# rhymes-ai/Aria

Hardware: NVIDIA H100
Metric: Aria-25.3B bf16 prefill tokens/sec (higher is better)
Workload: dtype bf16

## Files before the change

### aria_b200/csrc/gemm.cu

```cuda
#include <cuda_fp8.h>

#include "gemm_common.cuh"

namespace aria {

constexpr int GEMM_STAGES = 4;
constexpr int FP8_LAND_STAGES = 3;
constexpr int FP8_CONVERT_WARPS = 3;
constexpr int PAIR_MIN_ROWS = 2048;
constexpr int WIDE_PAIR_MIN_K = 2048;
template <int BN, bool B_FP8 = false>
constexpr int gemm_smem_bytes() {
  return 1024  + GEMM_STAGES * (A_STAGE_BYTES + BN * BK * 2) + BM * acc_ld(BN) * 4 + 256  +
         (B_FP8 ? FP8_LAND_STAGES * BN * BK : 0);
}
static_assert(gemm_smem_bytes<128, true>() <= 232448, "fp8 landing ring must fit the opt-in shared memory of a block");

ARIA_DEVICE void e4m3x16_to_bf16(const uint4 v, uint4& lo, uint4& hi) {
  const uint32_t w[4] = {v.x, v.y, v.z, v.w};
  uint32_t o[8];
#pragma unroll
  for (int i = 0; i < 4; ++i) {
#pragma unroll
    for (int h = 0; h < 2; ++h) {
      const __half2_raw hr = __nv_cvt_fp8x2_to_halfraw2(static_cast<__nv_fp8x2_storage_t>(w[i] >> (16 * h)), __NV_E4M3);
      const float2 f = __half22float2(__half2(hr));
      o[2 * i + h] = pack_bf16(f.x, f.y);
    }
  }
  lo = make_uint4(o[0], o[1], o[2], o[3]);
  hi = make_uint4(o[4], o[5], o[6], o[7]);
}

template <bool PAIR> ARIA_DEVICE int first_tile() { return PAIR ? blockIdx.x >> 1 : blockIdx.x; }
template <bool PAIR> ARIA_DEVICE int tile_step() { return PAIR ? gridDim.x >> 1 : gridDim.x; }
template <bool PAIR> ARIA_DEVICE int pair_sched_n(int n_tiles) { return PAIR ? (n_tiles + 1) / 2 : n_tiles; }

template <int BN, bool B_MN>
ARIA_DEVICE void wgmma_tile_k16(float (&acc)[BN / 2], uint64_t da, uint64_t db) {
  if constexpr (BN == 128) wgmma_m64n128_ss<0, B_MN ? 1 : 0>(acc, da, db, 1u);
  else wgmma_m64n144_ss<0, B_MN ? 1 : 0>(acc, da, db, 1u);
}

// ... 199 lines not shown
        const uint64_t db = db0 + rp.stage * (STAGE_BYTES >> 4);
        wgmma_fence();
#pragma unroll
        for (int k = 0; k < BK / 16; ++k) wgmma_tile_k16<BN, B_MN>(acc, da + k * 2, db + k * b_kadv);
        wgmma_commit();
        wgmma_wait<1>();
        if (prev >= 0) release(prev);
        prev = static_cast<int>(rp.stage);
        rp.next();
      }
      wgmma_wait<0>();
      fence_regs(acc);
      if (prev >= 0) release(prev);
      stage_and_epilogue<BN, EPI, B_FP8 ? AccScale::COL : AccScale::NONE>(p, stg, ct, acc, bsc, 1.f, 1.f, n_out_total, grp,
                                                                           m_idx, n_idx, row0, rows);
    }
  }
  if constexpr (PAIR) cluster_sync();
}

constexpr int WIDE_BN = 192;
constexpr int WIDE_STAGE_BYTES = A_STAGE_BYTES + WIDE_BN * BK * 2;
constexpr int WIDE_BOX_BYTES = 64 * 64 * 2;
constexpr int WIDE_HALF_BYTES = 3 * WIDE_BOX_BYTES;
constexpr int gemm_wide_smem_bytes() {
  return 1024  + GEMM_STAGES * WIDE_STAGE_BYTES + 2 * WIDE_HALF_BYTES + 256 ;
}
static_assert(gemm_wide_smem_bytes() <= 232448, "wide GEMM must fit the opt-in shared memory of a block");

ARIA_DEVICE uint32_t wide_out_offset(int r, int c) {
  return (c >> 6) * WIDE_BOX_BYTES + r * 128 + ((((c & 63) >> 3) ^ (r & 7)) << 4) + (c & 7) * 2;
}

template <int EPI, bool PAIR>
__global__ void __launch_bounds__(GEMM_THREADS, 1)
gemm_wide_kernel(const __grid_constant__ CUtensorMap tmA, const __grid_constant__ CUtensorMap tmB0,
                 const __grid_constant__ CUtensorMap tmB1, const __grid_constant__ CUtensorMap tmB2,
                 const __grid_constant__ CUtensorMap tmOut, const __grid_constant__ CUtensorMap tmRes, const GemmParams p) {
  constexpr int BN = WIDE_BN;
  constexpr int STAGES = GEMM_STAGES;
  static_assert(EPI == ARIA_EPI_LINEAR || EPI == ARIA_EPI_HEADS, "wide GEMM epilogues");

  uint8_t* smem = smem_1024();
  uint8_t* out_tile = smem + STAGES * WIDE_STAGE_BYTES;
  const BarrierRing<STAGES> bar(out_tile + 2 * WIDE_HALF_BYTES);
  uint64_t* res_full = bar.empty + STAGES;
  uint64_t* out_free = res_full + 2;

  const int warp = threadIdx.x >> 5;
  const int lane = threadIdx.x & 31;
  const int wg = threadIdx.x >> 7;
  const bool res = EPI == ARIA_EPI_LINEAR && p.residual != nullptr;

  if (warp == 0 && lane == 0) {
    prefetch_tmap(&tmA);
    prefetch_tmap(&tmB0);
    if (p.n_seg > 1) prefetch_tmap(&tmB1);
    if (p.n_seg > 2) prefetch_tmap(&tmB2);
    if (EPI == ARIA_EPI_LINEAR) prefetch_tmap(&tmOut);
    if (res) prefetch_tmap(&tmRes);
    bar.init(1, PAIR ? 2 * CONSUMER_WARPS : CONSUMER_WARPS);
    for (int h = 0; h < 2; ++h) {
      mbar_init(&res_full[h], 1);
      mbar_init(&out_free[h], 1);
    }
    fence_mbar_init();
  }
  if constexpr (PAIR) cluster_sync();
  else __syncthreads();

  const int n_out_total = p.N * p.n_seg;
  const int n_tiles = (n_out_total + BN - 1) / BN;
  const int k_blocks = (p.K + BK - 1) / BK;
  const uint32_t smem_base = smem_u32(smem);
  const uint32_t full0 = smem_u32(bar.full), empty0 = smem_u32(bar.empty);
  auto tile_boxes = [&](int col0) { return min(3, (n_out_total - col0 + 63) / 64); };

  if (wg == 0) {
    setmaxnreg_dec<56>();
    if (warp == 0 && elect_one()) {
      const uint32_t rank = PAIR ? cluster_ctarank() : 0;
      TileSched sched;
      sched.init(p, pair_sched_n<PAIR>(n_tiles));
      RingPos<STAGES> rp;
      uint32_t out_phase = 0;
      for (int t = first_tile<PAIR>();; t += tile_step<PAIR>()) {
        int grp, m_idx, n_idx, row0, rows;
        if (!sched.decode(t, grp, m_idx, n_idx, row0, rows)) break;
        if constexpr (PAIR) n_idx = 2 * n_idx + rank;
        const bool phantom = PAIR && n_idx >= n_tiles;
        const int a_row = m_idx * BM;
        const int a_half_row = a_row + (a_row + static_cast<int>(rank) * (BM / 2) < rows ? rank * (BM / 2) : 0);
        const int col0 = n_idx * BN;
        const int seg = col0 / p.N;
        const CUtensorMap* tb = seg == 0 ? &tmB0 : (seg == 1 ? &tmB1 : &tmB2);
        const int b_row = col0 - seg * p.N;
        const int res_kb = min(STAGES - 1, k_blocks - 1);
        for (int kb = 0; kb < k_blocks; ++kb) {
          const uint32_t fb = full0 + rp.stage * 8;
          const uint32_t sa = smem_base + rp.stage * WIDE_STAGE_BYTES;
          mbar_wait_addr(empty0 + rp.stage * 8, rp.phase ^ 1);
          if constexpr (PAIR) {
            mbar_arrive_expect_tx_addr(fb, phantom ? A_STAGE_BYTES : WIDE_STAGE_BYTES);
            tma_load_2d_multicast_addr(sa + rank * (A_STAGE_BYTES / 2), &tmA, fb, kb * BK, a_half_row, 0b11);
            if (phantom) {
              rp.next();
              continue;
            }
          } else {
            mbar_arrive_expect_tx_addr(fb, WIDE_STAGE_BYTES);
            tma_load_2d_addr(sa, &tmA, fb, kb * BK, a_row);
          }
          tma_load_2d_addr(sa + A_STAGE_BYTES, tb, fb, kb * BK, b_row);
          rp.next();
          if (res && kb == res_kb) {
            const int nbox = tile_boxes(col0);
            for (int h = 0; h < 2; ++h) {
              if (a_row + 64 * h >= rows) continue;
              mbar_wait(&out_free[h], (out_phase >> h) & 1);
              out_phase ^= 1u << h;
              mbar_arrive_expect_tx(&res_full[h], nbox * WIDE_BOX_BYTES);
              for (int c = 0; c < nbox; ++c)
                tma_load_2d(out_tile + h * WIDE_HALF_BYTES + c * WIDE_BOX_BYTES, &tmRes, &res_full[h], col0 + 64 * c,
                            a_row + 64 * h);
            }
          }
        }
      }
    }
  } else {
    setmaxnreg_inc<224>();
    const int cw = wg - 1;
    const uint64_t da0 = make_smem_desc(smem_base + cw * 64 * 128, 16, 1024);
    const uint64_t db0 = make_smem_desc(smem_base + A_STAGE_BYTES, 16, 1024);
    const ConsumerThread ct = consumer_thread(cw, lane);
    const int fr = ct.frag_row - 64 * cw;
    const bool leader = (threadIdx.x & 127) == 0;
    uint8_t* half = out_tile + cw * WIDE_HALF_BYTES;
    const uint32_t rank = PAIR ? cluster_ctarank() : 0;
    TileSched sched;
    sched.init(p, pair_sched_n<PAIR>(n_tiles));
    RingPos<STAGES> rp;
    uint32_t res_phase = 0;
    auto release = [&](int s) {
      if (lane == 0) {
        mbar_arrive(&bar.empty[s]);
        if constexpr (PAIR) mbar_arrive_cluster(&bar.empty[s], rank ^ 1);
      }
    };
    auto pass_tile = [&] {
      for (int kb = 0; kb < k_blocks; ++kb) {
        mbar_wait_addr(full0 + rp.stage * 8, rp.phase);
        release(rp.stage);
        rp.next();
      }
    };
    for (int t = first_tile<PAIR>();; t += tile_step<PAIR>()) {
      int grp, m_idx, n_idx, row0, rows;
      if (!sched.decode(t, grp, m_idx, n_idx, row0, rows)) break;
      if constexpr (PAIR) n_idx = 2 * n_idx + rank;
      if (sits_out((PAIR && n_idx >= n_tiles) || m_idx * BM + 64 * cw >= rows)) {
        pass_tile();
        continue;
      }
      const int col0 = n_idx * BN;
      const int seg = col0 / p.N;
      const int cseg0 = col0 - seg * p.N;
      const __nv_bfloat16* bias = p.bias[seg];
      uint32_t bias2[BN / 8];
#pragma unroll
      for (int j = 0; j < BN / 8; ++j) {
        const int c = cseg0 + 8 * j + ct.frag_col;
        bias2[j] = (bias && c < p.N) ? __ldg(reinterpret_cast<const uint32_t*>(bias + c)) : 0u;
      }
      float acc[BN / 2];
#pragma unroll
      for (int i = 0; i < BN / 2; ++i) acc[i] = 0.f;
      int prev = -1;
      for (int kb = 0; kb < k_blocks; ++kb) {
        mbar_wait_addr(full0 + rp.stage * 8, rp.phase);
        const uint64_t da = da0 + rp.stage * (WIDE_STAGE_BYTES >> 4);
        const uint64_t db = db0 + rp.stage * (WIDE_STAGE_BYTES >> 4);
        wgmma_fence();
#pragma unroll
        for (int k = 0; k < BK / 16; ++k) wgmma_m64n192_ss<0, 0>(acc, da + k * 2, db + k * 2, 1u);
        wgmma_commit();
        if (kb == 0 && leader) {
          bulk_wait_group_read<0>();
          if (res) mbar_arrive(&out_free[cw]);
        }
        wgmma_wait<1>();
        if (prev >= 0) release(prev);
        prev = static_cast<int>(rp.stage);
        rp.next();
      }
      wgmma_wait<0>();
      fence_regs(acc);
      if (prev >= 0) release(prev);
      if (res) {
        mbar_wait(&res_full[cw], res_phase);
        res_phase ^= 1;
      }
      named_bar_sync(1 + cw, 128);
#pragma unroll
      for (int j = 0; j < BN / 8; ++j) {
        const int c = 8 * j + ct.frag_col;
#pragma unroll
        for (int i = 0; i < 2; ++i) {
          uint32_t* dst = reinterpret_cast<uint32_t*>(half + wide_out_offset(fr + 8 * i, c));
          float x0 = acc[4 * j + 2 * i], x1 = acc[4 * j + 2 * i + 1];
          if (bias) {
            x0 += bf16_lo(bias2[j]);
            x1 += bf16_hi(bias2[j]);
          }
          if constexpr (EPI == ARIA_EPI_LINEAR) {
            x0 = bf16r(x0);
            x1 = bf16r(x1);
            if (p.act != ARIA_ACT_NONE) {
              x0 = bf16r(act_apply(x0, p.act));
              x1 = bf16r(act_apply(x1, p.act));
            }
            if (res) {
              const uint32_t r = *dst;
              x0 += bf16_lo(r);
              x1 += bf16_hi(r);
            }
          }
          *dst = pack_bf16(x0, x1);
        }
        if (j % 8 == 7) asm volatile("" ::: "memory");
      }
      if constexpr (EPI == ARIA_EPI_LINEAR) {
        fence_proxy_async_smem();
        named_bar_sync(1 + cw, 128);
        if (leader) {
          const int nbox = tile_boxes(col0);
          for (int c = 0; c < nbox; ++c)
            tma_store_2d_addr(&tmOut, smem_u32(half + c * WIDE_BOX_BYTES), col0 + 64 * c, m_idx * BM + 64 * cw);
          bulk_commit_group();
        }
      } else {
        named_bar_sync(1 + cw, 128);
        constexpr int CH = BN / 8;
#pragma unroll 1
        for (int i = threadIdx.x & 127; i < 64 * CH; i += 128) {
          const int r = i / CH, c = (i % CH) * 8;
          const int r_in_grp = m_idx * BM + 64 * cw + r;
          const int cs = cseg0 + c;
          if (r_in_grp >= rows || cs + 8 > p.N) continue;
          const uint4 v = *reinterpret_cast<const uint4*>(half + wide_out_offset(r, c));
          const int b = r_in_grp / p.rows_per_batch, tok = r_in_grp - b * p.rows_per_batch;
          const int head = cs / p.head_dim, d = cs - head * p.head_dim;
          *reinterpret_cast<uint4*>(p.out[seg] + b * p.stride_b + static_cast<int64_t>(p.pos0 + tok) * p.head_ld +
                                    head * p.stride_h + d) = v;
        }
      }
    }
    if (leader) bulk_wait_group_read<0>();
  }
  if constexpr (PAIR) cluster_sync();
}

constexpr int W8_BK = 128;
static_assert(BM * W8_BK == A_STAGE_BYTES, "W8A8 A stage = bf16 A stage");

struct W8a8DenseScales {
  const float* b[3];
};

template <int BN, int EPI>
ARIA_DEVICE void load_dense_col_scales(const GemmParams& p, const W8a8DenseScales& sc, int n_idx, int frag_col,
                                       float2 (&bsc)[BN / 8]) {
#pragma unroll
  for (int j = 0; j < BN / 8; ++j) {
    int col, seg;
    if constexpr (EPI == ARIA_EPI_SWIGLU) {
      seg = 8 * j < BN / 2 ? 0 : 1;
      col = n_idx * (BN / 2) + 8 * j - seg * (BN / 2) + frag_col;
    } else {
      seg = n_idx * BN / p.N;
      col = n_idx * BN - seg * p.N + 8 * j + frag_col;
    }
    const float* srow = seg == 0 ? sc.b[0] : (seg == 1 ? sc.b[1] : sc.b[2]);
    bsc[j] = col < p.N ? __ldg(reinterpret_cast<const float2*>(srow + col)) : make_float2(0.f, 0.f);
  }
}

template <int EPI, bool DENSE>
ARIA_DEVICE void w8a8_body(const CUtensorMap* tmA, const CUtensorMap* tmA_min, const CUtensorMap* tmB0, const CUtensorMap* tmB1,
                           const CUtensorMap* tmB2, const GemmParams& p, const float* __restrict__ a_scale,
                           const W8a8DenseScales& dsc) {
  constexpr int BN = 128;
  constexpr int STAGE_BYTES = A_STAGE_BYTES + BN * W8_BK;
  constexpr int STAGES = GEMM_STAGES;
  constexpr int ACC_LD = acc_ld(BN);
// ... 219 lines not shown
    ARIA_CHECK_ARG(d->n_seg == 1);
    ARIA_CHECK_ARG(d->k % BK == 0 || (d->num_groups == 1 && d->group_mod == 0));
    ARIA_CHECK_ARG(d->n % 64 == 0);
    ARIA_CHECK_ARG(d->epilogue != ARIA_EPI_HEADS);
  } else {
    ARIA_CHECK_ARG(d->num_groups == 1 || d->n_seg == 1);
    if (swiglu) ARIA_CHECK_ARG(d->n_seg == 2 && d->b[1]);
    if (b_gnk) ARIA_CHECK_ARG(d->n_seg == 1 && !swiglu && d->epilogue == ARIA_EPI_LINEAR && d->n % 128 == 0);
    else ARIA_CHECK_ARG(d->num_groups == 1);
  }
  if (d->num_groups > 1) ARIA_CHECK_ARG(d->group_offsets != nullptr);
  if (d->group_counts) ARIA_CHECK_ARG(d->group_offsets != nullptr);
  if (d->out_group_base) ARIA_CHECK_ARG(d->out_group_row0 != nullptr && d->epilogue == ARIA_EPI_LINEAR && d->group_offsets != nullptr);
  ARIA_CHECK_ARG(d->a_rows == 0 || d->a_rows >= d->m);

  int BN = 128;
  if (d->epilogue == ARIA_EPI_HEADS) {
    ARIA_CHECK_ARG(d->head_dim > 0 && d->head_dim % 8 == 0 && d->head_ld >= d->head_dim && d->n % d->head_dim == 0);
    if (d->rope_mask) ARIA_CHECK_ARG(d->head_dim == 128 && d->rope_cos && d->rope_sin);
    if (d->n % 128 != 0) {
      ARIA_CHECK_ARG(!d->rope_mask && d->n % 144 == 0);
      BN = 144;
    }
    for (int s = 0; s < d->n_seg; ++s) ARIA_CHECK_ARG(d->out[s] && d->b[s]);
  } else {
    if (swiglu) ARIA_CHECK_ARG(d->n % 64 == 0);
    if (d->n_seg > 1 && !swiglu) ARIA_CHECK_ARG(d->n % BN == 0);
  }

  const bool dense = !b_scale && d->b_layout == ARIA_B_NK && d->num_groups == 1 && !d->group_offsets;
  const bool wide = dense && d->m >= PAIR_MIN_ROWS && (d->n_seg == 1 || d->n % WIDE_BN == 0) &&
                    (d->epilogue == ARIA_EPI_HEADS ? !d->rope_mask : d->epilogue == ARIA_EPI_LINEAR);
  const bool wide_pair = wide && d->epilogue == ARIA_EPI_LINEAR && d->k >= WIDE_PAIR_MIN_K;
  const bool pair = !wide && dense && d->epilogue == ARIA_EPI_LINEAR && d->m >= PAIR_MIN_ROWS;
  const bool half_a = wide_pair || pair;

  CUtensorMap tmA, tmA_min, tmB[3];
  const uint64_t a_buf_rows = d->a_rows > 0 ? d->a_rows : d->m;
  int rc = make_tmap_2d(&tmA, d->a, d->k, a_buf_rows, d->lda * 2, BK, half_a ? BM / 2 : BM);
  if (rc) return rc;
  tmA_min = tmA;
  if (d->group_offsets) {
    rc = make_tmap_2d(&tmA_min, d->a, d->k, a_buf_rows, d->lda * 2, BK, A_BOX_MIN);
    if (rc) return rc;
  }
  if (b_mn) {
    const uint64_t ncols = swiglu ? 2 * d->n : d->n;
    const uint64_t n_weights = d->group_mod > 0 ? d->group_mod : (d->group_mod < 0 ? d->num_groups / (-d->group_mod) : d->num_groups);
    rc = b_scale ? make_tmap_2d(&tmB[0], d->b[0], ncols, n_weights * d->k, ncols, 64, BK, CU_TENSOR_MAP_SWIZZLE_NONE,
                                CU_TENSOR_MAP_DATA_TYPE_UINT8)
                 : make_tmap_2d(&tmB[0], d->b[0], ncols, n_weights * d->k, ncols * 2, 64, BK);
    if (rc) return rc;
    tmB[1] = tmB[0];
    tmB[2] = tmB[0];
  } else {
    const int nb = swiglu ? 2 : d->n_seg;
    const uint32_t box_rows = swiglu ? BN / 2 : (wide ? WIDE_BN : BN);
    for (int s = 0; s < 3; ++s) {
      const void* ptr = s < nb ? d->b[s] : d->b[0];
      const uint64_t b_rows = b_gnk ? static_cast<uint64_t>(d->group_mod > 0 ? d->group_mod : (d->group_mod < 0 ? d->num_groups / (-d->group_mod) : d->num_groups)) * d->n : d->n;
      rc = make_tmap_2d(&tmB[s], ptr, d->k, b_rows, d->k * 2, BK, box_rows);
      if (rc) return rc;
    }
  }

  const GemmParams p = gemm_params(d, b_scale);
  if (wide) {
    CUtensorMap tmOut = tmA, tmRes = tmA;
    const uint64_t n_out = d->n * d->n_seg;
    if (d->epilogue == ARIA_EPI_LINEAR) {
      rc = make_tmap_2d(&tmOut, d->out[0], n_out, d->m, d->ldo * 2, 64, 64);
      if (rc) return rc;
      if (d->residual) {
        rc = make_tmap_2d(&tmRes, d->residual, n_out, d->m, d->ldr * 2, 64, 64);
        if (rc) return rc;
      }
    }
    const int64_t m_tiles = (d->m + BM - 1) / BM, n_tiles = (n_out + WIDE_BN - 1) / WIDE_BN;
    if (wide_pair)
      return launch_persistent_pairs<gemm_wide_kernel<ARIA_EPI_LINEAR, true>>("gemm_wide_kernel", GEMM_THREADS,
                                                                              gemm_wide_smem_bytes(), (n_tiles + 1) / 2 * m_tiles,
                                                                              stream, tmA, tmB[0], tmB[1], tmB[2], tmOut, tmRes, p);
#define ARIA_LAUNCH_WIDE(EPI_)                                                                                                \
  return launch_persistent<gemm_wide_kernel<EPI_, false>>("gemm_wide_kernel", GEMM_THREADS, gemm_wide_smem_bytes(),         \
                                                          n_tiles * m_tiles, stream, tmA, tmB[0], tmB[1], tmB[2], tmOut, tmRes, p)
    if (d->epilogue == ARIA_EPI_HEADS) ARIA_LAUNCH_WIDE(ARIA_EPI_HEADS);
    ARIA_LAUNCH_WIDE(ARIA_EPI_LINEAR);
#undef ARIA_LAUNCH_WIDE
  }
  const int64_t tiles = max_tiles(d, BN, d->num_groups > 1 ? d->num_groups : 0);
  if (pair) {
    const int64_t m_tiles = (d->m + BM - 1) / BM, pairs = (tiles / m_tiles + 1) / 2 * m_tiles;
    return launch_persistent_pairs<gemm_kernel<128, false, ARIA_EPI_LINEAR, false, true>>(
        "gemm_kernel", GEMM_THREADS, gemm_smem_bytes<128>(), pairs, stream, tmA, tmA_min, tmB[0], tmB[1], tmB[2], p);
  }
#define ARIA_LAUNCH(BN_, MN_, EPI_, ...)                                                                                     \
  return launch_persistent<gemm_kernel<BN_, MN_, EPI_, ##__VA_ARGS__>>("gemm_kernel", GEMM_THREADS,                          \
                                                                       gemm_smem_bytes<BN_, ##__VA_ARGS__>(), tiles, stream, \
                                                                       tmA, tmA_min, tmB[0], tmB[1], tmB[2], p)
  if (b_scale) {
    if (swiglu) ARIA_LAUNCH(128, true, ARIA_EPI_SWIGLU, true);
    ARIA_LAUNCH(128, true, ARIA_EPI_LINEAR, true);
  }
  if (d->epilogue == ARIA_EPI_HEADS) {
    if (BN == 128) ARIA_LAUNCH(128, false, ARIA_EPI_HEADS);
    ARIA_LAUNCH(144, false, ARIA_EPI_HEADS);
  }
  if (swiglu) {
    if (b_mn) ARIA_LAUNCH(128, true, ARIA_EPI_SWIGLU);
    ARIA_LAUNCH(128, false, ARIA_EPI_SWIGLU);
  }
  if (b_mn) ARIA_LAUNCH(128, true, ARIA_EPI_LINEAR);
  ARIA_LAUNCH(128, false, ARIA_EPI_LINEAR);
#undef ARIA_LAUNCH
}

extern "C" int aria_gemm(const aria_gemm_desc_t* d, aria_stream_t stream) {
  return gemm_run(d, nullptr, reinterpret_cast<cudaStream_t>(stream));
}

// ... 112 lines not shown
```

### aria_b200/csrc/ptx.cuh

```cuda
#pragma once
#include <cuda.h>
#include <cuda_bf16.h>
#include <cuda_runtime.h>
#include <stdint.h>

namespace aria {

#define ARIA_DEVICE __device__ __forceinline__

ARIA_DEVICE uint32_t smem_u32(const void* p) { return static_cast<uint32_t>(__cvta_generic_to_shared(p)); }

ARIA_DEVICE uint32_t elect_one() {
  uint32_t pred = 0;
  asm volatile(
      "{\n\t.reg .pred P;\n\t"
      "elect.sync _|P, 0xffffffff;\n\t"
      "selp.b32 %0, 1, 0, P;\n\t}\n"
      : "=r"(pred));
  return pred;
}

ARIA_DEVICE void mbar_init(uint64_t* bar, uint32_t count) {
  asm volatile("mbarrier.init.shared::cta.b64 [%0], %1;" ::"r"(smem_u32(bar)), "r"(count));
}
ARIA_DEVICE void fence_mbar_init() { asm volatile("fence.mbarrier_init.release.cluster;" ::: "memory"); }
ARIA_DEVICE void fence_proxy_async_smem() { asm volatile("fence.proxy.async.shared::cta;" ::: "memory"); }

ARIA_DEVICE void mbar_arrive_expect_tx(uint64_t* bar, uint32_t bytes) {
  asm volatile("mbarrier.arrive.expect_tx.shared::cta.b64 _, [%0], %1;" ::"r"(smem_u32(bar)), "r"(bytes)
               : "memory");
}
ARIA_DEVICE void mbar_arrive(uint64_t* bar) {
  asm volatile("mbarrier.arrive.shared::cta.b64 _, [%0];" ::"r"(smem_u32(bar)) : "memory");
}
ARIA_DEVICE bool mbar_try_wait(uint64_t* bar, uint32_t parity) {
  uint32_t ok;
  asm volatile(
      "{\n\t.reg .pred P;\n\t"
      "mbarrier.try_wait.parity.shared::cta.b64 P, [%1], %2;\n\t"
      "selp.b32 %0, 1, 0, P;\n\t}\n"
      : "=r"(ok) : "r"(smem_u32(bar)), "r"(parity) : "memory");
  return ok != 0;
}
ARIA_DEVICE void mbar_wait_addr(uint32_t addr, uint32_t parity) {
  uint32_t ok = 0;
  long long t0 = 0;
  for (uint32_t spin = 0;; ++spin) {
    asm volatile(
        "{\n\t.reg .pred P;\n\t"
        "mbarrier.try_wait.parity.shared::cta.b64 P, [%1], %2;\n\t"
        "selp.b32 %0, 1, 0, P;\n\t}\n"
        : "=r"(ok) : "r"(addr), "r"(parity) : "memory");
    if (ok) return;
    if ((spin & 0xFFF) == 0xFFF) {
      const long long now = clock64();
      if (t0 == 0) t0 = now;
      if (now - t0 > 4000000000ll) __trap();
    }
  }
}
ARIA_DEVICE void mbar_wait(uint64_t* bar, uint32_t parity) { mbar_wait_addr(smem_u32(bar), parity); }
ARIA_DEVICE void mbar_arrive_expect_tx_addr(uint32_t bar_addr, uint32_t bytes) {
  asm volatile("mbarrier.arrive.expect_tx.shared::cta.b64 _, [%0], %1;" ::"r"(bar_addr), "r"(bytes) : "memory");
}
ARIA_DEVICE void mbar_arrive_cluster(uint64_t* bar, uint32_t cta) {
  asm volatile(
      "{\n\t.reg .b32 ra;\n\t"
      "mapa.shared::cluster.u32 ra, %0, %1;\n\t"
      "mbarrier.arrive.shared::cluster.b64 _, [ra];\n\t}\n" ::"r"(smem_u32(bar)), "r"(cta)
      : "memory");
}

ARIA_DEVICE uint32_t cluster_ctarank() {
  uint32_t r;
  asm volatile("mov.u32 %0, %%cluster_ctarank;" : "=r"(r));
  return r;
}
ARIA_DEVICE void cluster_sync() {
  asm volatile("barrier.cluster.arrive.release;\n\tbarrier.cluster.wait.acquire;" ::: "memory");
}

ARIA_DEVICE void tma_load_2d_addr(uint32_t dst, const CUtensorMap* m, uint32_t bar_addr, int c0, int c1) {
  asm volatile(
      "cp.async.bulk.tensor.2d.shared::cluster.global.mbarrier::complete_tx::bytes [%0], [%1, {%3, %4}], [%2];"
      ::"r"(dst), "l"(reinterpret_cast<uint64_t>(m)), "r"(bar_addr), "r"(c0), "r"(c1)
      : "memory");
}
ARIA_DEVICE void tma_load_2d_multicast_addr(uint32_t dst, const CUtensorMap* m, uint32_t bar_addr, int c0, int c1,
                                            uint16_t cta_mask) {
  asm volatile(
      "cp.async.bulk.tensor.2d.shared::cluster.global.mbarrier::complete_tx::bytes.multicast::cluster [%0], [%1, {%3, %4}], [%2], %5;"
      ::"r"(dst), "l"(reinterpret_cast<uint64_t>(m)), "r"(bar_addr), "r"(c0), "r"(c1), "h"(cta_mask)
      : "memory");
}
ARIA_DEVICE void tma_store_2d_addr(const CUtensorMap* m, uint32_t src, int c0, int c1) {
  asm volatile("cp.async.bulk.tensor.2d.global.shared::cta.bulk_group [%0, {%2, %3}], [%1];"
               ::"l"(reinterpret_cast<uint64_t>(m)), "r"(src), "r"(c0), "r"(c1)
               : "memory");
}
ARIA_DEVICE void bulk_commit_group() { asm volatile("cp.async.bulk.commit_group;" ::: "memory"); }
template <int N> ARIA_DEVICE void bulk_wait_group_read() { asm volatile("cp.async.bulk.wait_group.read %0;" ::"n"(N) : "memory"); }
ARIA_DEVICE void prefetch_tmap(const CUtensorMap* m) {
  asm volatile("prefetch.tensormap [%0];" ::"l"(reinterpret_cast<uint64_t>(m)) : "memory");
}
ARIA_DEVICE void tma_load_2d(void* dst, const CUtensorMap* m, uint64_t* bar, int c0, int c1) {
// ... 144 lines not shown
```

Baseline: 19230.

## Add ping-pong warpgroup GEMM kernel for wide dense projections with moderate K

Adds a persistent ping-pong GEMM kernel in which two consumer warpgroups alternate tiles. Each warpgroup computes a full 128x128 tile while the other runs its epilogue, with named barriers handing over mainloop turns. It is routed to wide dense GEMMs that don't qualify for the wide-pair path, have at least 2048 output columns, and have A up to 24MB. The aim is to hide epilogue cost (bias, activation, residual, TMA store) behind the tensor-core mainloop. In exchange it adds a new code path with more complex synchronisation and smaller N tiles than the existing wide kernel.

Measured after the change: 19640, median of 6. +2.1%, better.

```diff
diff --git a/aria_b200/csrc/gemm.cu b/aria_b200/csrc/gemm.cu
--- a/aria_b200/csrc/gemm.cu
+++ b/aria_b200/csrc/gemm.cu
@@ -1,4 +1,6 @@
 #include <cuda_fp8.h>
+
+#include <type_traits>
 
 #include "gemm_common.cuh"
 
@@ -9,6 +11,8 @@
 constexpr int FP8_CONVERT_WARPS = 3;
 constexpr int PAIR_MIN_ROWS = 2048;
 constexpr int WIDE_PAIR_MIN_K = 2048;
+constexpr int PINGPONG_MIN_COLS = 2048;
+constexpr int64_t PINGPONG_MAX_A_BYTES = 24 << 20;
 template <int BN, bool B_FP8 = false>
 constexpr int gemm_smem_bytes() {
   return 1024  + GEMM_STAGES * (A_STAGE_BYTES + BN * BK * 2) + BM * acc_ld(BN) * 4 + 256  +
@@ -503,6 +507,229 @@
   if constexpr (PAIR) cluster_sync();
 }
 
+constexpr int PP_BN = 128;
+constexpr int PP_STAGES = 5;
+constexpr int PP_STAGE_BYTES = A_STAGE_BYTES + PP_BN * BK * 2;
+constexpr int PP_TILE_BYTES = 2 * 2 * WIDE_BOX_BYTES;
+constexpr int PP_BAR_TURN = 3;
+constexpr int gemm_pingpong_smem_bytes() {
+  return 1024  + PP_STAGES * PP_STAGE_BYTES + 2 * PP_TILE_BYTES + 256 ;
+}
+static_assert(gemm_pingpong_smem_bytes() <= 232448, "ping-pong GEMM must fit the opt-in shared memory of a block");
+
+ARIA_DEVICE uint32_t pp_out_offset(int r, int c) { return (r >> 6) * (2 * WIDE_BOX_BYTES) + wide_out_offset(r & 63, c); }
+
+template <int EPI, int ACT>
+__global__ void __launch_bounds__(GEMM_THREADS, 1)
+gemm_pingpong_kernel(const __grid_constant__ CUtensorMap tmA, const __grid_constant__ CUtensorMap tmB0,
+                     const __grid_constant__ CUtensorMap tmB1, const __grid_constant__ CUtensorMap tmB2,
+                     const __grid_constant__ CUtensorMap tmOut, const __grid_constant__ CUtensorMap tmRes, const GemmParams p) {
+  constexpr int BN = PP_BN;
+  constexpr int STAGES = PP_STAGES;
+  static_assert(EPI == ARIA_EPI_LINEAR || (EPI == ARIA_EPI_HEADS && ACT == ARIA_ACT_NONE), "ping-pong GEMM epilogues");
+
+  uint8_t* smem = smem_1024();
+  uint8_t* out_tile = smem + STAGES * PP_STAGE_BYTES;
+  const BarrierRing<STAGES> bar(out_tile + 2 * PP_TILE_BYTES);
+  uint64_t* res_full = bar.empty + STAGES;
+  uint64_t* out_free = res_full + 2;
+
+  const int warp = threadIdx.x >> 5;
+  const int lane = threadIdx.x & 31;
+  const int wg = threadIdx.x >> 7;
+  const bool res = EPI == ARIA_EPI_LINEAR && p.residual != nullptr;
+
+  if (warp == 0 && lane == 0) {
+    prefetch_tmap(&tmA);
+    prefetch_tmap(&tmB0);
+    if (p.n_seg > 1) prefetch_tmap(&tmB1);
+    if (p.n_seg > 2) prefetch_tmap(&tmB2);
+    if (EPI == ARIA_EPI_LINEAR) prefetch_tmap(&tmOut);
+    if (res) prefetch_tmap(&tmRes);
+    bar.init(1, CONSUMER_WARPS / 2);
+    for (int w = 0; w < 2; ++w) {
+      mbar_init(&res_full[w], 1);
+      mbar_init(&out_free[w], 1);
+    }
+    fence_mbar_init();
+  }
+  __syncthreads();
+
+  const int n_out_total = p.N * p.n_seg;
+  const int m_tiles = (p.M + BM - 1) / BM;
+  const int tiles = (n_out_total + BN - 1) / BN * m_tiles;
+  const int k_blocks = (p.K + BK - 1) / BK;
+  const uint32_t smem_base = smem_u32(smem);
+  const uint32_t full0 = smem_u32(bar.full), empty0 = smem_u32(bar.empty);
+  auto tile_boxes = [&](int col0) { return min(2, (n_out_total - col0 + 63) / 64); };
+
+  if (wg == 0) {
+    setmaxnreg_dec<40>();
+    if (warp == 0 && elect_one()) {
+      RingPos<STAGES> rp;
+      uint32_t out_phase = 0;
+      for (int i = 0, t = blockIdx.x; t < tiles; ++i, t += gridDim.x) {
+        const int n_idx = t / m_tiles, m_idx = t - n_idx * m_tiles;
+        const int a_row = m_idx * BM;
+        const int halves = a_row + 64 < p.M ? 2 : 1;
+        const int col0 = n_idx * BN;
+        const int seg = col0 / p.N;
+        const CUtensorMap* tb = seg == 0 ? &tmB0 : (seg == 1 ? &tmB1 : &tmB2);
+        const int b_row = col0 - seg * p.N;
+        const int res_kb = min(STAGES - 1, k_blocks - 1);
+        for (int kb = 0; kb < k_blocks; ++kb) {
+          const uint32_t fb = full0 + rp.stage * 8;
+          const uint32_t sa = smem_base + rp.stage * PP_STAGE_BYTES;
+          mbar_wait_addr(empty0 + rp.stage * 8, rp.phase ^ 1);
+          mbar_arrive_expect_tx_addr(fb, PP_STAGE_BYTES);
+          tma_load_2d_addr(sa, &tmA, fb, kb * BK, a_row);
+          tma_load_2d_addr(sa + A_STAGE_BYTES, tb, fb, kb * BK, b_row);
+          rp.next();
+          if (res && kb == res_kb) {
+            const int w = i & 1, nbox = tile_boxes(col0);
+            mbar_wait(&out_free[w], (out_phase >> w) & 1);
+            out_phase ^= 1u << w;
+            mbar_arrive_expect_tx(&res_full[w], halves * nbox * WIDE_BOX_BYTES);
+            for (int h = 0; h < halves; ++h)
+              for (int c = 0; c < nbox; ++c)
+                tma_load_2d(out_tile + w * PP_TILE_BYTES + (2 * h + c) * WIDE_BOX_BYTES, &tmRes, &res_full[w],
+                            col0 + 64 * c, a_row + 64 * h);
+          }
+        }
+      }
+    }
+  } else {
+    setmaxnreg_inc<232>();
+    const int cw = wg - 1;
+    const uint64_t da0 = make_smem_desc(smem_base, 16, 1024);
+    const uint64_t db0 = make_smem_desc(smem_base + A_STAGE_BYTES, 16, 1024);
+    constexpr uint32_t A_HALF = (64 * 128) >> 4;
+    const ConsumerThread ct = consumer_thread(0, lane);
+    const int fr = ct.frag_row;
+    const bool leader = (threadIdx.x & 127) == 0;
+    const uint32_t tile = smem_u32(out_tile + cw * PP_TILE_BYTES);
+    RingPos<STAGES> rp;
+    auto release = [&](int s) {
+      if (lane == 0) mbar_arrive(&bar.empty[s]);
+    };
+    for (int i = 0, t = blockIdx.x; t < tiles; ++i, t += gridDim.x) {
+      if ((i & 1) != cw) {
+        for (int kb = 0; kb < k_blocks; ++kb) rp.next();
+        continue;
+      }
+      const int n_idx = t / m_tiles, m_idx = t - n_idx * m_tiles;
+      const bool hi = m_idx * BM + 64 < p.M;
+      const int col0 = n_idx * BN;
+      const int seg = col0 / p.N;
+      const int cseg0 = col0 - seg * p.N;
+      float acc[2][BN / 2];
+#pragma unroll
+      for (int h = 0; h < 2; ++h)
+#pragma unroll
+        for (int j = 0; j < BN / 2; ++j) acc[h][j] = 0.f;
+      if (i > 0) named_bar_sync(PP_BAR_TURN + cw, 256);
+      auto mainloop = [&](auto HI) {
+        int prev = -1;
+        for (int kb = 0; kb < k_blocks; ++kb) {
+          mbar_wait_addr(full0 + rp.stage * 8, rp.phase);
+          const uint64_t da = da0 + rp.stage * (PP_STAGE_BYTES >> 4);
+          const uint64_t db = db0 + rp.stage * (PP_STAGE_BYTES >> 4);
+          wgmma_fence();
+#pragma unroll
+          for (int k = 0; k < BK / 16; ++k) {
+            wgmma_m64n128_ss<0, 0>(acc[0], da + k * 2, db + k * 2, 1u);
+            if constexpr (decltype(HI)::value) wgmma_m64n128_ss<0, 0>(acc[1], da + A_HALF + k * 2, db + k * 2, 1u);
+          }
+          wgmma_commit();
+          if (kb == 0 && leader) {
+            bulk_wait_group_read<0>();
+            if (res) mbar_arrive(&out_free[cw]);
+          }
+          wgmma_wait<1>();
+          if (prev >= 0) release(prev);
+          prev = static_cast<int>(rp.stage);
+          rp.next();
+        }
+        if (t + static_cast<int>(gridDim.x) < tiles) named_bar_arrive(PP_BAR_TURN + (cw ^ 1), 256);
+        wgmma_wait<0>();
+        fence_regs(acc[0]);
+        fence_regs(acc[1]);
+        if (prev >= 0) release(prev);
+      };
+      if (hi) mainloop(std::true_type{});
+      else mainloop(std::false_type{});
+      const __nv_bfloat16* bias = p.bias[seg];
+      uint32_t bias2[BN / 8];
+#pragma unroll
+      for (int j = 0; j < BN / 8; ++j) {
+        const int c = cseg0 + 8 * j + ct.frag_col;
+        bias2[j] = (bias && c < p.N) ? __ldg(reinterpret_cast<const uint32_t*>(bias + c)) : 0u;
+      }
+      if (res) mbar_wait(&res_full[cw], (i >> 1) & 1);
+      named_bar_sync(1 + cw, 128);
+#pragma unroll
+      for (int h = 0; h < 2; ++h) {
+        if (h == 1 && !hi) break;
+#pragma unroll
+        for (int j = 0; j < BN / 8; ++j) {
+          const int c = 8 * j + ct.frag_col;
+#pragma unroll
+          for (int e = 0; e < 2; ++e) {
+            const uint32_t dst = tile + pp_out_offset(64 * h + fr + 8 * e, c);
+            float x0 = acc[h][4 * j + 2 * e], x1 = acc[h][4 * j + 2 * e + 1];
+            if (bias) {
+              x0 += bf16_lo(bias2[j]);
+              x1 += bf16_hi(bias2[j]);
+            }
+            if constexpr (EPI == ARIA_EPI_LINEAR) {
+              bf16r2(x0, x1);
+              if constexpr (ACT != ARIA_ACT_NONE) {
+                x0 = act_apply(x0, ACT);
+                x1 = act_apply(x1, ACT);
+                bf16r2(x0, x1);
+              }
+              if (res) {
+                const uint32_t r = ld_shared_b32(dst);
+                x0 += bf16_lo(r);
+                x1 += bf16_hi(r);
+              }
+            }
+            st_shared_b32(dst, pack_bf16(x0, x1));
+          }
+          if (j % 8 == 7) asm volatile("" ::: "memory");
+        }
+      }
+      if constexpr (EPI == ARIA_EPI_LINEAR) {
+        fence_proxy_async_smem();
+        named_bar_sync(1 + cw, 128);
+        if (leader) {
+          const int nbox = tile_boxes(col0);
+          for (int h = 0; h < (hi ? 2 : 1); ++h)
+            for (int c = 0; c < nbox; ++c)
+              tma_store_2d_addr(&tmOut, tile + (2 * h + c) * WIDE_BOX_BYTES, col0 + 64 * c, m_idx * BM + 64 * h);
+          bulk_commit_group();
+        }
+      } else {
+        named_bar_sync(1 + cw, 128);
+        constexpr int CH = BN / 8;
+#pragma unroll 1
+        for (int q = threadIdx.x & 127; q < BM * CH; q += 128) {
+          const int r = q / CH, c = (q % CH) * 8;
+          const int r_in_grp = m_idx * BM + r;
+          const int cs = cseg0 + c;
+          if (r_in_grp >= p.M || cs + 8 > p.N) continue;
+          const uint4 v = ld_shared_v4(tile + pp_out_offset(r, c));
+          const int b = r_in_grp / p.rows_per_batch, tok = r_in_grp - b * p.rows_per_batch;
+          const int head = cs / p.head_dim, d = cs - head * p.head_dim;
+          *reinterpret_cast<uint4*>(p.out[seg] + b * p.stride_b + static_cast<int64_t>(p.pos0 + tok) * p.head_ld +
+                                    head * p.stride_h + d) = v;
+        }
+      }
+    }
+    if (leader) bulk_wait_group_read<0>();
+  }
+}
+
 constexpr int W8_BK = 128;
 static_assert(BM * W8_BK == A_STAGE_BYTES, "W8A8 A stage = bf16 A stage");
 
@@ -788,6 +1015,8 @@
   const bool wide = dense && d->m >= PAIR_MIN_ROWS && (d->n_seg == 1 || d->n % WIDE_BN == 0) &&
                     (d->epilogue == ARIA_EPI_HEADS ? !d->rope_mask : d->epilogue == ARIA_EPI_LINEAR);
   const bool wide_pair = wide && d->epilogue == ARIA_EPI_LINEAR && d->k >= WIDE_PAIR_MIN_K;
+  const bool pingpong = wide && !wide_pair && d->n * d->n_seg >= PINGPONG_MIN_COLS && (d->n_seg == 1 || d->n % PP_BN == 0) &&
+                        d->m * d->k * 2 <= PINGPONG_MAX_A_BYTES;
   const bool pair = !wide && dense && d->epilogue == ARIA_EPI_LINEAR && d->m >= PAIR_MIN_ROWS;
   const bool half_a = wide_pair || pair;
 
@@ -811,7 +1040,7 @@
     tmB[2] = tmB[0];
   } else {
     const int nb = swiglu ? 2 : d->n_seg;
-    const uint32_t box_rows = swiglu ? BN / 2 : (wide ? WIDE_BN : BN);
+    const uint32_t box_rows = swiglu ? BN / 2 : (pingpong ? PP_BN : (wide ? WIDE_BN : BN));
     for (int s = 0; s < 3; ++s) {
       const void* ptr = s < nb ? d->b[s] : d->b[0];
       const uint64_t b_rows = b_gnk ? static_cast<uint64_t>(d->group_mod > 0 ? d->group_mod : (d->group_mod < 0 ? d->num_groups / (-d->group_mod) : d->num_groups)) * d->n : d->n;
@@ -833,6 +1062,17 @@
       }
     }
     const int64_t m_tiles = (d->m + BM - 1) / BM, n_tiles = (n_out + WIDE_BN - 1) / WIDE_BN;
+    if (pingpong) {
+      const int64_t tiles = (n_out + PP_BN - 1) / PP_BN * m_tiles;
+#define ARIA_LAUNCH_PP(EPI_, ACT_)                                                                                             \
+  return launch_persistent<gemm_pingpong_kernel<EPI_, ACT_>>("gemm_pingpong_kernel", GEMM_THREADS, gemm_pingpong_smem_bytes(), \
+                                                             tiles, stream, tmA, tmB[0], tmB[1], tmB[2], tmOut, tmRes, p)
+      if (d->epilogue == ARIA_EPI_HEADS) ARIA_LAUNCH_PP(ARIA_EPI_HEADS, ARIA_ACT_NONE);
+      if (d->act == ARIA_ACT_GELU_TANH) ARIA_LAUNCH_PP(ARIA_EPI_LINEAR, ARIA_ACT_GELU_TANH);
+      if (d->act == ARIA_ACT_GELU_NEW) ARIA_LAUNCH_PP(ARIA_EPI_LINEAR, ARIA_ACT_GELU_NEW);
+      ARIA_LAUNCH_PP(ARIA_EPI_LINEAR, ARIA_ACT_NONE);
+#undef ARIA_LAUNCH_PP
+    }
     if (wide_pair)
       return launch_persistent_pairs<gemm_wide_kernel<ARIA_EPI_LINEAR, true>>("gemm_wide_kernel", GEMM_THREADS,
                                                                               gemm_wide_smem_bytes(), (n_tiles + 1) / 2 * m_tiles,
diff --git a/aria_b200/csrc/ptx.cuh b/aria_b200/csrc/ptx.cuh
--- a/aria_b200/csrc/ptx.cuh
+++ b/aria_b200/csrc/ptx.cuh
@@ -71,6 +71,18 @@
       : "memory");
 }
 
+ARIA_DEVICE void st_shared_b32(uint32_t addr, uint32_t v) { asm volatile("st.shared.b32 [%0], %1;" ::"r"(addr), "r"(v)); }
+ARIA_DEVICE uint32_t ld_shared_b32(uint32_t addr) {
+  uint32_t v;
+  asm volatile("ld.shared.b32 %0, [%1];" : "=r"(v) : "r"(addr));
+  return v;
+}
+ARIA_DEVICE uint4 ld_shared_v4(uint32_t addr) {
+  uint4 v;
+  asm volatile("ld.shared.v4.b32 {%0, %1, %2, %3}, [%4];" : "=r"(v.x), "=r"(v.y), "=r"(v.z), "=r"(v.w) : "r"(addr));
+  return v;
+}
+
 ARIA_DEVICE uint32_t cluster_ctarank() {
   uint32_t r;
   asm volatile("mov.u32 %0, %%cluster_ctarank;" : "=r"(r));
```

## Hand off wide GEMM epilogue to idle producer warps via out_full barriers

Applied to the files above, without the earlier changes.

For wide GEMM launches without a residual, the consumer warpgroups now only write bias-added bf16 accumulators into the shared-memory output tile and signal an out_full barrier. The three otherwise idle producer-warpgroup warps then apply GELU in place, issue the TMA stores, or scatter the HEADS layout to global memory. The aim is to overlap epilogue work (activation, stores) with the next tile's MMA main loop. In exchange it adds barrier round-trips and makes consumers wait on out_free before writing. Epilogue throughput is limited to 96 threads running with a reduced register budget. GELU is now applied to the bf16-rounded stored value, which matches the old rounding order.

Measured after the change: 19270 before, 19860 after (median of 6 runs). +3.1%, better.

```diff
diff --git a/aria_b200/csrc/gemm.cu b/aria_b200/csrc/gemm.cu
--- a/aria_b200/csrc/gemm.cu
+++ b/aria_b200/csrc/gemm.cu
@@ -274,7 +274,29 @@
   return (c >> 6) * WIDE_BOX_BYTES + r * 128 + ((((c & 63) >> 3) ^ (r & 7)) << 4) + (c & 7) * 2;
 }
 
-template <int EPI, bool PAIR>
+constexpr int WIDE_EPI_THREADS = 96;
+constexpr uint32_t WIDE_EPI_BAR = 3;
+
+template <int ACT>
+ARIA_DEVICE void wide_act_inplace(uint32_t half, int n_chunks, int et) {
+  auto act8 = [](uint4& v) {
+    uint32_t* w = reinterpret_cast<uint32_t*>(&v);
+#pragma unroll
+    for (int e = 0; e < 4; ++e) w[e] = pack_bf16(bf16r(act_apply(bf16_lo(w[e]), ACT)), bf16r(act_apply(bf16_hi(w[e]), ACT)));
+  };
+#pragma unroll 1
+  for (int i = et; i < n_chunks; i += 2 * WIDE_EPI_THREADS) {
+    const uint32_t a0 = half + 16 * i, a1 = a0 + 16 * WIDE_EPI_THREADS;
+    const bool two = i + WIDE_EPI_THREADS < n_chunks;
+    uint4 v0 = ld_shared_v4(a0), v1 = two ? ld_shared_v4(a1) : make_uint4(0, 0, 0, 0);
+    act8(v0);
+    act8(v1);
+    st_shared_v4(a0, v0);
+    if (two) st_shared_v4(a1, v1);
+  }
+}
+
+template <int EPI, bool PAIR, bool HANDOFF>
 __global__ void __launch_bounds__(GEMM_THREADS, 1)
 gemm_wide_kernel(const __grid_constant__ CUtensorMap tmA, const __grid_constant__ CUtensorMap tmB0,
                  const __grid_constant__ CUtensorMap tmB1, const __grid_constant__ CUtensorMap tmB2,
@@ -282,17 +304,20 @@
   constexpr int BN = WIDE_BN;
   constexpr int STAGES = GEMM_STAGES;
   static_assert(EPI == ARIA_EPI_LINEAR || EPI == ARIA_EPI_HEADS, "wide GEMM epilogues");
+  static_assert(HANDOFF || EPI == ARIA_EPI_LINEAR, "HEADS launches hand off");
 
   uint8_t* smem = smem_1024();
   uint8_t* out_tile = smem + STAGES * WIDE_STAGE_BYTES;
   const BarrierRing<STAGES> bar(out_tile + 2 * WIDE_HALF_BYTES);
   uint64_t* res_full = bar.empty + STAGES;
   uint64_t* out_free = res_full + 2;
+  uint64_t* out_full = out_free + 2;
 
   const int warp = threadIdx.x >> 5;
   const int lane = threadIdx.x & 31;
   const int wg = threadIdx.x >> 7;
-  const bool res = EPI == ARIA_EPI_LINEAR && p.residual != nullptr;
+  constexpr bool handoff = HANDOFF;
+  constexpr bool res = !HANDOFF;
 
   if (warp == 0 && lane == 0) {
     prefetch_tmap(&tmA);
@@ -305,6 +330,7 @@
     for (int h = 0; h < 2; ++h) {
       mbar_init(&res_full[h], 1);
       mbar_init(&out_free[h], 1);
+      mbar_init(&out_full[h], 128);
     }
     fence_mbar_init();
   }
@@ -369,6 +395,64 @@
           }
         }
       }
+    } else if (warp > 0 && handoff) {
+      const int et = threadIdx.x - 32;
+      const uint32_t rank = PAIR ? cluster_ctarank() : 0;
+      TileSched sched;
+      sched.init(p, pair_sched_n<PAIR>(n_tiles));
+      uint32_t full_phase = 0;
+      for (int t = first_tile<PAIR>();; t += tile_step<PAIR>()) {
+        int grp, m_idx, n_idx, row0, rows;
+        if (!sched.decode(t, grp, m_idx, n_idx, row0, rows)) break;
+        if constexpr (PAIR) n_idx = 2 * n_idx + rank;
+        if (PAIR && n_idx >= n_tiles) continue;
+        const int col0 = n_idx * BN;
+        const int seg = col0 / p.N;
+        const int cseg0 = col0 - seg * p.N;
+        for (int h = 0; h < 2; ++h) {
+          if (m_idx * BM + 64 * h >= rows) continue;
+          mbar_wait(&out_full[h], (full_phase >> h) & 1);
+          full_phase ^= 1u << h;
+          const uint32_t half = smem_u32(out_tile) + h * WIDE_HALF_BYTES;
+          if constexpr (EPI == ARIA_EPI_LINEAR) {
+            const int nbox = tile_boxes(col0);
+            if (p.act == ARIA_ACT_GELU_TANH || p.act == ARIA_ACT_GELU_NEW) {
+              const int n_chunks = nbox * (WIDE_BOX_BYTES / 16);
+              if (p.act == ARIA_ACT_GELU_TANH) wide_act_inplace<ARIA_ACT_GELU_TANH>(half, n_chunks, et);
+              else wide_act_inplace<ARIA_ACT_GELU_NEW>(half, n_chunks, et);
+              fence_proxy_async_smem();
+            }
+            named_bar_sync(WIDE_EPI_BAR, WIDE_EPI_THREADS);
+            if (et == 0) {
+              fence_proxy_async_smem();
+              for (int c = 0; c < nbox; ++c)
+                tma_store_2d_addr(&tmOut, half + c * WIDE_BOX_BYTES, col0 + 64 * c, m_idx * BM + 64 * h);
+              bulk_commit_group();
+              bulk_wait_group_read<0>();
+              mbar_arrive(&out_free[h]);
+            }
+          } else {
+            constexpr int CH = BN / 8;
+            constexpr int ROW_STEP = WIDE_EPI_THREADS / CH;
+            static_assert(WIDE_EPI_THREADS % CH == 0, "a thread keeps its column chunk");
+            const int c = (et % CH) * 8, cs = cseg0 + c;
+            if (cs + 8 <= p.N) {
+              const int head = cs / p.head_dim, d = cs - head * p.head_dim;
+              __nv_bfloat16* col_base = p.out[seg] + head * p.stride_h + d;
+              int r = et / CH, r_in_grp = m_idx * BM + 64 * h + r;
+              int b = r_in_grp / p.rows_per_batch, tok = r_in_grp - b * p.rows_per_batch;
+#pragma unroll 1
+              for (; r < 64 && r_in_grp < rows; r += ROW_STEP, r_in_grp += ROW_STEP) {
+                st_global_v4(col_base + b * p.stride_b + static_cast<int64_t>(p.pos0 + tok) * p.head_ld,
+                             ld_shared_v4(half + wide_out_offset(r, c)));
+                for (tok += ROW_STEP; tok >= p.rows_per_batch; tok -= p.rows_per_batch) ++b;
+              }
+            }
+            named_bar_sync(WIDE_EPI_BAR, WIDE_EPI_THREADS);
+            if (et == 0) mbar_arrive(&out_free[h]);
+          }
+        }
+      }
     }
   } else {
     setmaxnreg_inc<224>();
@@ -379,11 +463,12 @@
     const int fr = ct.frag_row - 64 * cw;
     const bool leader = (threadIdx.x & 127) == 0;
     uint8_t* half = out_tile + cw * WIDE_HALF_BYTES;
+    const uint32_t half_s = smem_u32(half);
     const uint32_t rank = PAIR ? cluster_ctarank() : 0;
     TileSched sched;
     sched.init(p, pair_sched_n<PAIR>(n_tiles));
     RingPos<STAGES> rp;
-    uint32_t res_phase = 0;
+    uint32_t res_phase = 0, free_phase = 0;
     auto release = [&](int s) {
       if (lane == 0) {
         mbar_arrive(&bar.empty[s]);
@@ -427,9 +512,9 @@
 #pragma unroll
         for (int k = 0; k < BK / 16; ++k) wgmma_m64n192_ss<0, 0>(acc, da + k * 2, db + k * 2, 1u);
         wgmma_commit();
-        if (kb == 0 && leader) {
+        if (res && kb == 0 && leader) {
           bulk_wait_group_read<0>();
-          if (res) mbar_arrive(&out_free[cw]);
+          mbar_arrive(&out_free[cw]);
         }
         wgmma_wait<1>();
         if (prev >= 0) release(prev);
@@ -439,40 +524,53 @@
       wgmma_wait<0>();
       fence_regs(acc);
       if (prev >= 0) release(prev);
-      if (res) {
+      if (handoff) {
+        mbar_wait(&out_free[cw], free_phase ^ 1);
+        free_phase ^= 1;
+#pragma unroll
+        for (int j = 0; j < BN / 8; ++j) {
+#pragma unroll
+          for (int i = 0; i < 2; ++i) {
+            float x0 = acc[4 * j + 2 * i], x1 = acc[4 * j + 2 * i + 1];
+            if (bias) {
+              x0 += bf16_lo(bias2[j]);
+              x1 += bf16_hi(bias2[j]);
+            }
+            st_shared_u32(half_s + wide_out_offset(fr + 8 * i, 8 * j + ct.frag_col), pack_bf16(x0, x1));
+          }
+        }
+        if constexpr (EPI == ARIA_EPI_LINEAR) fence_proxy_async_smem();
+        mbar_arrive(&out_full[cw]);
+        continue;
+      }
+      if constexpr (EPI == ARIA_EPI_LINEAR) {
         mbar_wait(&res_full[cw], res_phase);
         res_phase ^= 1;
-      }
-      named_bar_sync(1 + cw, 128);
-#pragma unroll
-      for (int j = 0; j < BN / 8; ++j) {
-        const int c = 8 * j + ct.frag_col;
-#pragma unroll
-        for (int i = 0; i < 2; ++i) {
-          uint32_t* dst = reinterpret_cast<uint32_t*>(half + wide_out_offset(fr + 8 * i, c));
-          float x0 = acc[4 * j + 2 * i], x1 = acc[4 * j + 2 * i + 1];
-          if (bias) {
-            x0 += bf16_lo(bias2[j]);
-            x1 += bf16_hi(bias2[j]);
-          }
-          if constexpr (EPI == ARIA_EPI_LINEAR) {
+        named_bar_sync(1 + cw, 128);
+#pragma unroll
+        for (int j = 0; j < BN / 8; ++j) {
+          const int c = 8 * j + ct.frag_col;
+#pragma unroll
+          for (int i = 0; i < 2; ++i) {
+            uint32_t* dst = reinterpret_cast<uint32_t*>(half + wide_out_offset(fr + 8 * i, c));
+            float x0 = acc[4 * j + 2 * i], x1 = acc[4 * j + 2 * i + 1];
+            if (bias) {
+              x0 += bf16_lo(bias2[j]);
+              x1 += bf16_hi(bias2[j]);
+            }
             x0 = bf16r(x0);
             x1 = bf16r(x1);
             if (p.act != ARIA_ACT_NONE) {
               x0 = bf16r(act_apply(x0, p.act));
               x1 = bf16r(act_apply(x1, p.act));
             }
-            if (res) {
-              const uint32_t r = *dst;
-              x0 += bf16_lo(r);
-              x1 += bf16_hi(r);
-            }
+            const uint32_t r = *dst;
+            x0 += bf16_lo(r);
+            x1 += bf16_hi(r);
+            *dst = pack_bf16(x0, x1);
           }
-          *dst = pack_bf16(x0, x1);
-        }
-        if (j % 8 == 7) asm volatile("" ::: "memory");
-      }
-      if constexpr (EPI == ARIA_EPI_LINEAR) {
+          if (j % 8 == 7) asm volatile("" ::: "memory");
+        }
         fence_proxy_async_smem();
         named_bar_sync(1 + cw, 128);
         if (leader) {
@@ -480,21 +578,6 @@
           for (int c = 0; c < nbox; ++c)
             tma_store_2d_addr(&tmOut, smem_u32(half + c * WIDE_BOX_BYTES), col0 + 64 * c, m_idx * BM + 64 * cw);
           bulk_commit_group();
-        }
-      } else {
-        named_bar_sync(1 + cw, 128);
-        constexpr int CH = BN / 8;
-#pragma unroll 1
-        for (int i = threadIdx.x & 127; i < 64 * CH; i += 128) {
-          const int r = i / CH, c = (i % CH) * 8;
-          const int r_in_grp = m_idx * BM + 64 * cw + r;
-          const int cs = cseg0 + c;
-          if (r_in_grp >= rows || cs + 8 > p.N) continue;
-          const uint4 v = *reinterpret_cast<const uint4*>(half + wide_out_offset(r, c));
-          const int b = r_in_grp / p.rows_per_batch, tok = r_in_grp - b * p.rows_per_batch;
-          const int head = cs / p.head_dim, d = cs - head * p.head_dim;
-          *reinterpret_cast<uint4*>(p.out[seg] + b * p.stride_b + static_cast<int64_t>(p.pos0 + tok) * p.head_ld +
-                                    head * p.stride_h + d) = v;
         }
       }
     }
@@ -833,15 +916,21 @@
       }
     }
     const int64_t m_tiles = (d->m + BM - 1) / BM, n_tiles = (n_out + WIDE_BN - 1) / WIDE_BN;
-    if (wide_pair)
-      return launch_persistent_pairs<gemm_wide_kernel<ARIA_EPI_LINEAR, true>>("gemm_wide_kernel", GEMM_THREADS,
-                                                                              gemm_wide_smem_bytes(), (n_tiles + 1) / 2 * m_tiles,
-                                                                              stream, tmA, tmB[0], tmB[1], tmB[2], tmOut, tmRes, p);
-#define ARIA_LAUNCH_WIDE(EPI_)                                                                                                \
-  return launch_persistent<gemm_wide_kernel<EPI_, false>>("gemm_wide_kernel", GEMM_THREADS, gemm_wide_smem_bytes(),         \
-                                                          n_tiles * m_tiles, stream, tmA, tmB[0], tmB[1], tmB[2], tmOut, tmRes, p)
-    if (d->epilogue == ARIA_EPI_HEADS) ARIA_LAUNCH_WIDE(ARIA_EPI_HEADS);
-    ARIA_LAUNCH_WIDE(ARIA_EPI_LINEAR);
+    if (wide_pair) {
+      const int64_t pairs = (n_tiles + 1) / 2 * m_tiles;
+      if (d->residual)
+        return launch_persistent_pairs<gemm_wide_kernel<ARIA_EPI_LINEAR, true, false>>(
+            "gemm_wide_kernel", GEMM_THREADS, gemm_wide_smem_bytes(), pairs, stream, tmA, tmB[0], tmB[1], tmB[2], tmOut, tmRes, p);
+      return launch_persistent_pairs<gemm_wide_kernel<ARIA_EPI_LINEAR, true, true>>(
+          "gemm_wide_kernel", GEMM_THREADS, gemm_wide_smem_bytes(), pairs, stream, tmA, tmB[0], tmB[1], tmB[2], tmOut, tmRes, p);
+    }
+#define ARIA_LAUNCH_WIDE(EPI_, HANDOFF_)                                                                                      \
+  return launch_persistent<gemm_wide_kernel<EPI_, false, HANDOFF_>>("gemm_wide_kernel", GEMM_THREADS, gemm_wide_smem_bytes(), \
+                                                                    n_tiles * m_tiles, stream, tmA, tmB[0], tmB[1], tmB[2],   \
+                                                                    tmOut, tmRes, p)
+    if (d->epilogue == ARIA_EPI_HEADS) ARIA_LAUNCH_WIDE(ARIA_EPI_HEADS, true);
+    if (d->residual) ARIA_LAUNCH_WIDE(ARIA_EPI_LINEAR, false);
+    ARIA_LAUNCH_WIDE(ARIA_EPI_LINEAR, true);
 #undef ARIA_LAUNCH_WIDE
   }
   const int64_t tiles = max_tiles(d, BN, d->num_groups > 1 ? d->num_groups : 0);
diff --git a/aria_b200/csrc/ptx.cuh b/aria_b200/csrc/ptx.cuh
--- a/aria_b200/csrc/ptx.cuh
+++ b/aria_b200/csrc/ptx.cuh
@@ -9,6 +9,18 @@
 #define ARIA_DEVICE __device__ __forceinline__
 
 ARIA_DEVICE uint32_t smem_u32(const void* p) { return static_cast<uint32_t>(__cvta_generic_to_shared(p)); }
+ARIA_DEVICE void st_shared_u32(uint32_t addr, uint32_t v) { asm volatile("st.shared.b32 [%0], %1;" ::"r"(addr), "r"(v) : "memory"); }
+ARIA_DEVICE void st_shared_v4(uint32_t addr, uint4 v) {
+  asm volatile("st.shared.v4.b32 [%0], {%1, %2, %3, %4};" ::"r"(addr), "r"(v.x), "r"(v.y), "r"(v.z), "r"(v.w) : "memory");
+}
+ARIA_DEVICE void st_global_v4(void* p, uint4 v) {
+  asm volatile("st.global.v4.b32 [%0], {%1, %2, %3, %4};" ::"l"(p), "r"(v.x), "r"(v.y), "r"(v.z), "r"(v.w) : "memory");
+}
+ARIA_DEVICE uint4 ld_shared_v4(uint32_t addr) {
+  uint4 v;
+  asm volatile("ld.shared.v4.b32 {%0, %1, %2, %3}, [%4];" : "=r"(v.x), "=r"(v.y), "=r"(v.z), "=r"(v.w) : "r"(addr) : "memory");
+  return v;
+}
 
 ARIA_DEVICE uint32_t elect_one() {
   uint32_t pred = 0;
```
